# facebookresearch/dmc-net

Measured on AMD Instinct MI355X. Metric: clips/sec (3-seg 224x224) DMC-gen+ResNet-18 train step, higher is better.
Workload: dtype f32

## Files before the change

### dmc-net_amd/csrc/conv_x3q.hip

```cpp
#include "dmc_common.h"
#include "x3s_common.h"
#include <type_traits>
#include <utility>

using namespace dmc;
using namespace dmc::x3;

namespace {

constexpr int QBM = 256, QBN = 64;
constexpr int QWSLOT = 3 * QBN * 32;
constexpr int QWB = 3 * QWSLOT;
constexpr int QEP = 272, QETILE = 32 * QEP;

template <int NW_, int NPB_, int NT_>
struct QG {
    static constexpr int NW = NW_, NPB = NPB_, NT = NT_;
    static constexpr int NA = NW / 2;
    static constexpr int KP = (NT + NA - 1) / NA;
    static constexpr int PT = 3 * KP;
    static constexpr int KW = (18 + NA - 1) / NA;
    static constexpr int ZROW = 32 * NT;
    static constexpr int PSL = (ZROW + 1) * 32;
    static constexpr int PB = 3 * PSL;
// ... 453 lines not shown

template <int TN, class GEO>
int launch_q_eval(const X3qEvalArgs& a, hipStream_t s) {
    static LdsLimit lim;
    const hipError_t attr = lim.raise(reinterpret_cast<const void*>(&x3q_conv_kernel<ProgFwd, TN, GEO, true>), GEO::LDS);
    if (attr != hipSuccess) return fail(DMC_E_LAUNCH, "x3q_conv_bn_eval: cannot raise the dynamic LDS limit: %s", hipGetErrorString(attr));
    constexpr int BM = 32 * GEO::NW / (2 / TN);
    dim3 grid((a.M + BM - 1) / BM, a.R / QBN);
    x3q_conv_kernel<ProgFwd, TN, GEO, true><<<grid, GEO::NW * 64, GEO::LDS, s>>>(a);
    return check_launch("x3q_conv_bn_eval");
}

int q_patch_pixels_max128(long M, int W);
int q_variant(long M, int W, int R) {
    const int forced = option(OPT_CONV_CFG);
    const bool two_ok = q_patch_pixels_max128(M, W) <= QGTwo::ZROW;
    if (forced == 201) return 0;
    if (forced == 202) return 1;
    if (forced == 203 && two_ok) return 2;
    if (forced != 204 && two_ok && ((M + 127) / 128) * (R / QBN) >= 512) return 2;
    return q_choose_tn(M, R) == 2 ? 0 : 1;
}
int q_block_pixels(int variant) { return variant == 0 ? 256 : 128; }


struct X3qWgArgs {
    const void* xq;
    const void* dys;
    float* part;
    int N, OH, Cin, Cout;
    unsigned plane_bytes;
    int steps, per_group, tiles_ci;
};

template <int OW_, int R, int HP_>
struct QWgGeom {
    static constexpr int PW = OW_ + 1;
    static constexpr int D1 = 3, D0 = 2;
    static constexpr int XPL1 = ((D1 * R * PW + 3) / 8) * 8 + 4;
    static constexpr int XPL0 = ((D0 * R * PW + 3) / 8) * 8 + 4;
    static constexpr int NPX = R * OW_;
    static constexpr int NKB = (NPX + 15) / 16;
    static constexpr int DYT = ((NKB * 16 + 31) / 32) * 32;
    static constexpr int DYPL = ((DYT + 3) / 8) * 8 + 4;
    static constexpr int XI = (R * PW + 31) / 32;
    static constexpr int DI = DYT / 32;
    static constexpr int CLS_OFF[4] = {0, 4 * XPL0 * 32, 8 * XPL0 * 32, 8 * XPL0 * 32 + 4 * XPL1 * 32};
    static constexpr int SLB = 8 * XPL0 * 32 + 8 * XPL1 * 32;
    static constexpr int XBYTES = 3 * SLB, DYBYTES = 12 * DYPL * 32;
    static constexpr int LDS = XBYTES + 2 * DYBYTES;
    static_assert(HP_ % R == 0, "steps are whole groups of padded rows");
};

template <int OW_, int R, int HP_>
__global__ __launch_bounds__(768) void x3q_wgrad_kernel(X3qWgArgs a) {
    using G = QWgGeom<OW_, R, HP_>;
    constexpr int PW = G::PW, DYPL = G::DYPL, NKB = G::NKB;
    extern __shared__ __attribute__((aligned(1024))) char lds_qw[];
    const int tid = threadIdx.x, lane = tid & 63;
    const int wave = __builtin_amdgcn_readfirstlane(tid >> 6);
    const int l31 = lane & 31, khalf = lane >> 5, L = lane & 15, grp = (lane >> 4) & 1;
    const int quarter = wave & 3, trow = wave >> 2;
    const int wi = quarter & 1, wj = quarter >> 1;
    const int tci = blockIdx.x % a.tiles_ci, tco = blockIdx.x / a.tiles_ci;
    const unsigned lds0 = lds_addr_of(lds_qw);
    const int s_begin = blockIdx.y * a.per_group;
    const int s_end = s_begin + a.per_group < a.steps ? s_begin + a.per_group : a.steps;
    const u32x4 srd_x = make_srd(a.xq), srd_d = make_srd(a.dys);
    const int nch_in = a.Cin >> 4;
    const int tsl = wave >> 2, tch = wave & 3;
    const unsigned soff_d = (unsigned)(tsl * (a.Cout >> 4) + tco * 4 + tch) * a.plane_bytes;
    const unsigned dplane = lds0 + G::XBYTES + (unsigned)wave * DYPL * 32;
    const int lpx = lane >> 1;
    const unsigned lhalf = (unsigned)(lane & 1) << 4;

    const unsigned img_bytes = (unsigned)(a.OH * OW_) * 32u;
    unsigned xpre[G::XI], dpre[G::DI];
#pragma unroll
    for (int i = 0; i < G::XI; ++i) {
        const int px = 32 * i + lpx;
        const int r = px / PW, col = px - r * PW - 1;
        xpre[i] = (col >= 0 && col < OW_) ? (unsigned)(r * OW_ + col) * 32u + lhalf : NOPIX;
    }
#pragma unroll
    for (int i = 0; i < G::DI; ++i) {
        const int p = 32 * i + lpx;
        dpre[i] = p < G::NPX ? (unsigned)p * 32u + lhalf : NOPIX;
    }
    auto issue_x = [&](int q, const WgGroupPos& g) {
        unsigned tbase, img_off;
        wg_group_base(g, a.N, OW_, img_bytes, tbase, img_off);
        unsigned voff[G::XI];
#pragma unroll
        for (int i = 0; i < G::XI; ++i) voff[i] = wg_lane_off(tbase, xpre[i], img_bytes);
#pragma unroll
        for (int cls = 0; cls < 4; ++cls) {
            const int D = (cls >> 1) ? G::D1 : G::D0, xpl = (cls >> 1) ? G::XPL1 : G::XPL0;
            const int slot0 = (((q % D) + D) % D) * R;
            const unsigned soff_x = (unsigned)(tsl * 4 * nch_in + cls * nch_in + tci * 4 + tch) * a.plane_bytes + img_off;
            const unsigned xplane = lds0 + (unsigned)(tsl * G::SLB + G::CLS_OFF[cls] + tch * xpl * 32);
#pragma unroll
            for (int i = 0; i < G::XI; ++i)
                if (32 * i + lpx < R * PW) dma_buf16(srd_x, voff[i], soff_x, xplane + (unsigned)(slot0 * PW + 32 * i) * 32u);
        }
    };
    auto issue_dy = [&](const WgGroupPos& g, int buf) {
        unsigned tbase, img_off;
        wg_group_base(g, a.N, OW_, img_bytes, tbase, img_off);
#pragma unroll
        for (int i = 0; i < G::DI; ++i)
            dma_buf16(srd_d, wg_lane_off(tbase, dpre[i], img_bytes), soff_d + img_off, dplane + (unsigned)buf * G::DYBYTES + (unsigned)(32 * i) * 32u);
    };

    f32x16 acc[3];
#pragma unroll
    for (int t = 0; t < 3; ++t)
#pragma unroll
        for (int e = 0; e < 16; ++e) acc[t][e] = 0.f;

    WgGroupPos g1 = wg_group_at(s_begin, R, HP_);
    if (s_begin < s_end) {
        issue_x(s_begin - 1, wg_group_prev(g1, R, HP_));
        issue_x(s_begin, g1);
        issue_dy(g1, 0);
    }
    g1 = wg_group_next(g1, R, HP_);
    asm volatile("s_waitcnt vmcnt(0)" ::: "memory");
    __builtin_amdgcn_s_barrier();
    const int py = trow != 1, da = trow == 0 ? -1 : 0;
    const int DR = (py ? G::D1 : G::D0) * R, xpl = py ? G::XPL1 : G::XPL0;
    const int cls_a = py ? G::CLS_OFF[3] : G::CLS_OFF[1];
    const int cls_b = py ? G::CLS_OFF[2] : G::CLS_OFF[0];
    lds_cptr const LB = (lds_cptr)lds_qw;
    int rr[NKB][2], xcol[NKB][2], dyoff[NKB][2];
#pragma unroll
    for (int kb = 0; kb < NKB; ++kb)
#pragma unroll
        for (int u = 0; u < 2; ++u) {
            int P = 16 * kb + 8 * khalf + 4 * u + (L >> 2);
            dyoff[kb][u] = (2 * wi + grp) * DYPL * 32 + G::XBYTES + (L & 3) * 8 + P * 32;
            if (P >= G::NPX) P = G::NPX - 1;
            rr[kb][u] = P / OW_;
            xcol[kb][u] = (2 * wj + grp) * xpl * 32 + (L & 3) * 8 + (P - rr[kb][u] * OW_) * 32;
        }
#pragma unroll 1
    for (int s = s_begin; s < s_end; ++s) {
        const int buf = (s - s_begin) & 1;
        issue_x(s + 1, g1);
        if (s + 1 < s_end) issue_dy(g1, buf ^ 1);
        g1 = wg_group_next(g1, R, HP_);
        const int sb = (((R * s + da) % DR) + DR) % DR;
#pragma unroll
        for (int kb = 0; kb < NKB; ++kb) {
            int dyo[2], xa[2], xb[2];
#pragma unroll
            for (int u = 0; u < 2; ++u) {
                dyo[u] = dyoff[kb][u] + buf * G::DYBYTES;
                int slot = sb + rr[kb][u];
                slot = slot >= DR ? slot - DR : slot;
                const int xo = xcol[kb][u] + slot * PW * 32;
                xa[u] = xo + cls_a;
                xb[u] = xo + cls_b;
            }
            u32x4 A[3], B[3][3];
#pragma unroll
            for (int sl = 0; sl < 3; ++sl) {
                A[sl] = tr_read2(LB + dyo[0] + sl * 4 * DYPL * 32, LB + dyo[1] + sl * 4 * DYPL * 32);
                B[0][sl] = tr_read2(LB + xa[0] + sl * G::SLB, LB + xa[1] + sl * G::SLB);
                B[1][sl] = tr_read2(LB + xb[0] + sl * G::SLB + 32, LB + xb[1] + sl * G::SLB + 32);
                B[2][sl] = tr_read2(LB + xa[0] + sl * G::SLB + 32, LB + xa[1] + sl * G::SLB + 32);
            }
#pragma unroll
            for (int t = 0; t < 3; ++t) {
                acc[t] = mfma_bf16(A[0], B[t][2], acc[t]);
                acc[t] = mfma_bf16(A[2], B[t][0], acc[t]);
                acc[t] = mfma_bf16(A[1], B[t][1], acc[t]);
                acc[t] = mfma_bf16(A[0], B[t][1], acc[t]);
                acc[t] = mfma_bf16(A[1], B[t][0], acc[t]);
                acc[t] = mfma_bf16(A[0], B[t][0], acc[t]);
            }
        }
        asm volatile("s_waitcnt vmcnt(0) lgkmcnt(0)" ::: "memory");
        __builtin_amdgcn_s_barrier();
    }
    float* out = a.part + (size_t)blockIdx.y * a.Cout * 9 * a.Cin;
    const int ci = tci * 64 + 32 * wj + l31;
#pragma unroll
    for (int t = 0; t < 3; ++t)
#pragma unroll
        for (int e = 0; e < 16; ++e) {
            const int co = tco * 64 + 32 * wi + 8 * (e >> 2) + 4 * khalf + (e & 3);
            out[((size_t)co * 9 + 3 * trow + t) * a.Cin + ci] = acc[t][e];
        }
}

struct X3qWg1Args {
    const void* xq; const void* dys; float* part;
    int Cin, Cout; long Mq; unsigned plane_bytes; int steps, per_group, tiles_ci;
};
constexpr int W1PX = 64, W1PL = 68;
constexpr int W1TILE = 12 * W1PL * 32, W1LDS = 4 * W1TILE;

__global__ __launch_bounds__(256) void x3q_wgrad1_kernel(X3qWg1Args a) {
    extern __shared__ __attribute__((aligned(1024))) char lds_w1[];
    const int tid = threadIdx.x, lane = tid & 63;
    const int wave = __builtin_amdgcn_readfirstlane(tid >> 6);
    const int l31 = lane & 31, khalf = lane >> 5, L = lane & 15, grp = (lane >> 4) & 1;
    const int wi = wave & 1, wj = wave >> 1;
    const int tci = blockIdx.x % a.tiles_ci, tco = blockIdx.x / a.tiles_ci;
    const unsigned lds0 = lds_addr_of(lds_w1);
    const int s_begin = blockIdx.y * a.per_group;
    const int s_end = s_begin + a.per_group < a.steps ? s_begin + a.per_group : a.steps;
    const u32x4 srd_x = make_srd(a.xq), srd_d = make_srd(a.dys);
    const int nch_in = a.Cin >> 4, nch_out = a.Cout >> 4;
    const int lpx = lane >> 1;
    const unsigned lhalf = (unsigned)(lane & 1) << 4;
    auto issue = [&](int s, int buf) {
#pragma unroll
        for (int k = 0; k < 3; ++k) {
            const int pl = 3 * wave + k, sl = pl >> 2, ch = pl & 3;
#pragma unroll
            for (int i = 0; i < 2; ++i) {
                const long p = (long)s * W1PX + 32 * i + lpx;
                const unsigned voff = p < a.Mq ? (unsigned)p * 32u + lhalf : OOB;
                dma_buf16(srd_x, voff, (unsigned)(sl * 4 * nch_in + tci * 4 + ch) * a.plane_bytes,
                          lds0 + (unsigned)(buf * 2 * W1TILE + pl * W1PL * 32 + 32 * i * 32));
                dma_buf16(srd_d, voff, (unsigned)(sl * nch_out + tco * 4 + ch) * a.plane_bytes,
                          lds0 + (unsigned)(buf * 2 * W1TILE + W1TILE + pl * W1PL * 32 + 32 * i * 32));
            }
        }
    };
    f32x16 acc;
#pragma unroll
    for (int e = 0; e < 16; ++e) acc[e] = 0.f;
    if (s_begin < s_end) issue(s_begin, 0);
    asm volatile("s_waitcnt vmcnt(0)" ::: "memory");
// ... 11 lines not shown
            const int P0 = 16 * kb + 8 * khalf + (L >> 2), P1 = P0 + 4;
#pragma unroll
            for (int sl = 0; sl < 3; ++sl) {
                A[sl] = tr_read2(LB + db + sl * 4 * W1PL * 32 + P0 * 32, LB + db + sl * 4 * W1PL * 32 + P1 * 32);
                B[sl] = tr_read2(LB + xb + sl * 4 * W1PL * 32 + P0 * 32, LB + xb + sl * 4 * W1PL * 32 + P1 * 32);
            }
            acc = mfma_bf16(A[0], B[2], acc);
            acc = mfma_bf16(A[2], B[0], acc);
            acc = mfma_bf16(A[1], B[1], acc);
            acc = mfma_bf16(A[0], B[1], acc);
            acc = mfma_bf16(A[1], B[0], acc);
            acc = mfma_bf16(A[0], B[0], acc);
        }
        asm volatile("s_waitcnt vmcnt(0) lgkmcnt(0)" ::: "memory");
        __builtin_amdgcn_s_barrier();
    }
    float* out = a.part + (size_t)blockIdx.y * a.Cout * a.Cin;
    const int ci = tci * 64 + 32 * wj + l31;
#pragma unroll
    for (int e = 0; e < 16; ++e) {
        const int co = tco * 64 + 32 * wi + 8 * (e >> 2) + 4 * khalf + (e & 3);
        out[(size_t)co * a.Cin + ci] = acc[e];
    }
}

__global__ __launch_bounds__(256) void x3q_wgrad_reduce_kernel(const float* __restrict__ part, float* __restrict__ dw, int ngroup, long numel) {
    for (long i0 = (long)blockIdx.x * 64; i0 < numel; i0 += (long)gridDim.x * 64) wgrad_reduce_step(part, dw, ngroup, numel, i0);
}

struct QWgPlan { int R, HP, steps, tiles, groups, per_group, steps1, groups1, per_group1; };
bool q_wgrad_plan(int N, int OH, int OW, int Cin, int Cout, QWgPlan& p) {
    if (Cin % 64 != 0 || Cout % 64 != 0 || N <= 0) return false;
    if (OW == 28 && OH == 28) { p.R = 1; p.HP = 29; }
    else if (OW == 14 && OH == 14) { p.R = 2; p.HP = 16; }
    else if (OW == 7 && OH == 7) { p.R = 4; p.HP = 8; }
    else return false;
    p.steps = N * p.HP / p.R;
    p.tiles = (Cout / 64) * (Cin / 64);
    int groups = 256 / p.tiles;
    if (groups < 1) groups = 1;
    if (groups > p.steps) groups = p.steps;
    p.per_group = (p.steps + groups - 1) / groups;
    p.groups = (p.steps + p.per_group - 1) / p.per_group;
    const long Mq = (long)N * OH * OW;
    p.steps1 = (int)((Mq + W1PX - 1) / W1PX);
    int g1 = 512 / p.tiles;
    if (g1 < 1) g1 = 1;
    if (g1 > p.steps1) g1 = p.steps1;
    p.per_group1 = (p.steps1 + g1 - 1) / g1;
    p.groups1 = (p.steps1 + p.per_group1 - 1) / p.per_group1;
    return true;
}

template <int OW_, int R, int HP_>
int launch_q_wgrad(const QWgPlan& p, const X3qWgArgs& a, hipStream_t s) {
    using G = QWgGeom<OW_, R, HP_>;
    static_assert(G::LDS <= 160 * 1024, "weight-gradient tiles exceed the LDS");
    static LdsLimit lim;
    const hipError_t attr = lim.raise(reinterpret_cast<const void*>(&x3q_wgrad_kernel<OW_, R, HP_>), G::LDS);
    if (attr != hipSuccess) return fail(DMC_E_LAUNCH, "x3q_wgrad: cannot raise the dynamic LDS limit: %s", hipGetErrorString(attr));
    x3q_wgrad_kernel<OW_, R, HP_><<<dim3(p.tiles, p.groups), 768, G::LDS, s>>>(a);
    return check_launch("x3q_wgrad");
}

}

extern "C" {

size_t dmc_x3q_wpack_bytes(int Cin, int Cout) { return (size_t)Cin * (size_t)Cout * 10 * 6; }

int dmc_x3q_supported(int N, int OH, int OW, int Cin, int Cout) { return q_shape_ok(N, OH, OW, Cin, Cout) ? 1 : 0; }

int dmc_x3q_stat_blocks(int N, int OH, int OW, int Cout) {
    const long M = (long)N * OH * OW;
    const int bm = q_block_pixels(q_variant(M, OW, Cout));
    return (int)((M + bm - 1) / bm);
}

int dmc_x3q_split(const float* x, void* xq, int N, int H, int W, int C, dmc_stream_t stream) {
    if (!x || !xq || N <= 0 || H <= 0 || W <= 0 || (H & 1) || (W & 1) || C <= 0 || C % 16 != 0)
        return fail(DMC_E_INVALID, "dmc_x3q_split: bad argument");
    x3q_split_kernel<<<stream_blocks_q((long)N * H * W * (C / 8)), 256, 0, (hipStream_t)stream>>>(x, static_cast<unsigned short*>(xq), N, H, W, C);
    return check_launch("x3q_split");
}

int dmc_x3q_merge(const void* xq, float* x, int N, int H, int W, int C, dmc_stream_t stream) {
    if (!x || !xq || N <= 0 || H <= 0 || W <= 0 || (H & 1) || (W & 1) || C <= 0 || C % 16 != 0)
        return fail(DMC_E_INVALID, "dmc_x3q_merge: bad argument");
    x3q_merge_kernel<<<stream_blocks_q((long)N * H * W * C), 256, 0, (hipStream_t)stream>>>(static_cast<const unsigned short*>(xq), x, N, H, W, C);
    return check_launch("x3q_merge");
}

int dmc_x3q_pack_weights(const float* w3, const float* w1, void* wpack_f, void* wpack_t, int Cin, int Cout, dmc_stream_t stream) {
    if (!w3 || !w1 || (!wpack_f && !wpack_t) || Cin % 64 != 0 || Cout % 64 != 0 || Cin <= 0 || Cout <= 0)
        return fail(DMC_E_INVALID, "dmc_x3q_pack_weights: bad argument");
    const long total = (long)Cin * Cout * 10;
    const int blocks = stream_blocks_q(total) > 1024 ? 1024 : stream_blocks_q(total);
    x3q_pack_w_kernel<<<dim3(blocks, 2), 256, 0, (hipStream_t)stream>>>(w3, w1, static_cast<unsigned short*>(wpack_f),
                                                                           static_cast<unsigned short*>(wpack_t), Cout, Cin);
    return check_launch("x3q_pack_w");
}

int dmc_x3q_conv_fwd(const void* xq, const void* wpack_f, float* y3, float* y1, double* stat_partials3, double* stat_partials1,
                     int stat_blocks, int N, int OH, int OW, int Cin, int Cout, dmc_stream_t stream) {
    if (!xq || !wpack_f || !y3 || !y1) return fail(DMC_E_INVALID, "dmc_x3q_conv_fwd: null pointer");
    if (!q_shape_ok(N, OH, OW, Cin, Cout))
        return fail(DMC_E_INVALID, "dmc_x3q_conv_fwd: unsupported shape N=%d OH=%d OW=%d Cin=%d Cout=%d", N, OH, OW, Cin, Cout);
    const int var = q_variant((long)N * OH * OW, OW, Cout);
    const int rows = (int)(((long)N * OH * OW + q_block_pixels(var) - 1) / q_block_pixels(var));
    if ((stat_partials3 || stat_partials1) && stat_blocks != rows)
        return fail(DMC_E_INVALID, "dmc_x3q_conv_fwd: statistics partials have %d rows but this launch writes %d (dmc_x3q_stat_blocks "
                                   "was called under another conv_cfg option?)", stat_blocks, rows);
    X3qArgs a;
    a.t0 = xq; a.t1 = nullptr; a.wp = wpack_f; a.y0 = y3; a.y1 = y1; a.part0 = stat_partials3; a.part1 = stat_partials1;
    a.N = N; a.H = OH; a.W = OW; a.K = Cin; a.R = Cout; a.M = N * OH * OW;
// ... 89 lines not shown
```

### dmc-net_amd/csrc/conv_x3s.hip

```cpp
#include "dmc_common.h"
#include "x3s_common.h"
#include <type_traits>

using namespace dmc;
using namespace dmc::x3;

namespace {

__global__ __launch_bounds__(256) void x3s_split_kernel(const float* __restrict__ x, unsigned short* __restrict__ xs, long M, int C) {
    const int c8 = C >> 3;
    const long total = M * c8;
    const int nchunk = C >> 4;
    for (long o = (long)blockIdx.x * 256 + threadIdx.x; o < total; o += (long)gridDim.x * 256) {
        const long m = o / c8;
        const int g = (int)(o - m * c8);
        const float4 a = reinterpret_cast<const float4*>(x)[2 * o], b = reinterpret_cast<const float4*>(x)[2 * o + 1];
        const float v[8] = {a.x, a.y, a.z, a.w, b.x, b.y, b.z, b.w};
        x3s_store8(xs, v, (size_t)M, nchunk, (size_t)m, g);
    }
}

__global__ __launch_bounds__(256) void x3s_merge_kernel(const unsigned short* __restrict__ xs, float* __restrict__ x, long M, int C) {
    const long total = M * C;
    const size_t plane = (size_t)M * 16;
// ... 574 lines not shown
}

struct X3Bnb { const float *y, *stats, *gamma, *beta; const unsigned char* mask; int relu; double* part; };

int run_x3s(const void* xs, const void* wp, const float* addend, float* y, double* stat_part, int part_blocks, int N, int H, int W,
            int K, int R, hipStream_t s, const X3Bnb* bnb = nullptr) {
    if (!xs || !wp || !y) return fail(DMC_E_INVALID, "x3s_conv: null pointer");
    if (!x3s_shape_ok(N, H, W, K, R)) return fail(DMC_E_INVALID, "x3s_conv: unsupported shape N=%d H=%d W=%d K=%d R=%d", N, H, W, K, R);
    const int cfg = x3s_choose(N, H, W, R);
    X3Args a;
    a.xs = xs; a.wp = wp; a.y = y; a.addend = addend; a.stat_part = stat_part;
    a.N = N; a.H = H; a.W = W; a.K = K; a.R = R; a.M = N * H * W;
    a.plane_bytes = (unsigned)a.M * 32u;
    a.part_blocks = part_blocks;
    a.bms = cfg >= 0 ? x3s_tile_stride(cfg, W) : 0;
    if ((stat_part || bnb) && part_blocks <= 0) return fail(DMC_E_INVALID, "x3s_conv: stat_blocks must be the row count of the partials");
    if (bnb) {
        a.bnb_y = bnb->y; a.bnb_stats = bnb->stats; a.bnb_gamma = bnb->gamma; a.bnb_beta = bnb->beta; a.bnb_mask = bnb->mask;
        a.bnb_relu = bnb->relu; a.bnb_part = bnb->part;
    }
    a.ablate = option(OPT_CONV_ABLATE);
    if (DMC_ABL(a.ablate) & 32) a.stat_part = nullptr;
    switch (cfg) {
        case 0: return launch_x3s<8, 1, 608>(a, s);
        case 1: return launch_x3s<4, 1, 320>(a, s);
        case 2: return launch_x3s<2, 1, 192>(a, s);
        case 3: return launch_x3s<4, 2, 608>(a, s);
        case 4: return launch_x3s<4, 1, 225>(a, s);
        case 5: return launch_x3s<8, 2, 640, true>(a, s);
        default: return fail(DMC_E_INVALID, "x3s_conv: the patch of a %d x %d image does not fit the LDS", H, W);
    }
}

template <int WM, int TM, int PPMAX, bool ROWT = false>
int launch_x3s_eval(const X3EvalArgs& a, hipStream_t s) {
    constexpr int BM = 32 * TM * WM;
    constexpr size_t lds_bytes = 2 * 3 * PPMAX * 32 + 2 * 3 * 3 * 64 * 32;
    static_assert((size_t)BM * 272 <= lds_bytes && lds_bytes <= 160 * 1024, "the epilogue tiles live in the operand LDS");
    dim3 grid((a.M + a.bms - 1) / a.bms, a.R / 64);
    static LdsLimit lim_attr;
    const hipError_t attr = lim_attr.raise(reinterpret_cast<const void*>(&x3s_conv_kernel<WM, 1, TM, 2, PPMAX, (WM >= 4), 1, true, ROWT>), (int)lds_bytes);
    if (attr != hipSuccess) return fail(DMC_E_LAUNCH, "x3s_conv_bn_eval: cannot raise the dynamic LDS limit: %s", hipGetErrorString(attr));
    x3s_conv_kernel<WM, 1, TM, 2, PPMAX, (WM >= 4), 1, true, ROWT><<<grid, WM * 64, lds_bytes, s>>>(a);
    return check_launch("x3s_conv_bn_eval");
}

struct X3WgArgs {
    const void* xs;
    const void* dys;
    float* part;
    int N, H, Cin, Cout;
    unsigned plane_bytes;
    int steps, per_group, tiles_ci;
};

template <int W_, int R>
struct WgGeom {
    static constexpr int PW = W_ + 2;
    static constexpr int NGRP = R >= W_ + 2 ? 2 : 4, LA = NGRP / 2;
    static constexpr int NRING = NGRP * R;
    static constexpr int XPX = NRING * PW;
    static constexpr int XPL = ((XPX + 3) / 8) * 8 + 4;
    static constexpr int NPX = R * W_;
    static constexpr int NKB = (NPX + 15) / 16;
    static constexpr int DYP = NKB * 16;
    static constexpr int DYT = ((DYP + 31) / 32) * 32;
    static constexpr int DYPL = ((DYT + 3) / 8) * 8 + 4;
    static constexpr int XI = (R * PW + 31) / 32;
    static constexpr int DI = DYT / 32;
    static constexpr int XBYTES = 12 * XPL * 32, DYBYTES = 12 * DYPL * 32;
    static constexpr int LDS = XBYTES + 2 * DYBYTES;
};

template <int W_, int R>
__global__ __launch_bounds__(768) void x3s_wgrad_kernel(X3WgArgs a) {
    using G = WgGeom<W_, R>;
    constexpr int PW = G::PW, NRING = G::NRING, XPL = G::XPL, DYPL = G::DYPL, NKB = G::NKB;
    extern __shared__ __attribute__((aligned(1024))) char lds_wg[];
    const int tid = threadIdx.x, lane = tid & 63;
    const int wave = __builtin_amdgcn_readfirstlane(tid >> 6);
    const int l31 = lane & 31, khalf = lane >> 5, L = lane & 15, grp = (lane >> 4) & 1;
    const int quarter = wave & 3, trow = wave >> 2;
    const int wi = quarter & 1, wj = quarter >> 1;
    const int tci = blockIdx.x % a.tiles_ci, tco = blockIdx.x / a.tiles_ci;
    const unsigned lds0 = lds_addr_of(lds_wg);
    const int HP = a.H + 2;
    const int s_begin = blockIdx.y * a.per_group;
    const int s_end = s_begin + a.per_group < a.steps ? s_begin + a.per_group : a.steps;
    const u32x4 srd_x = make_srd(a.xs), srd_d = make_srd(a.dys);
    const unsigned soff_x = (unsigned)((wave >> 2) * (a.Cin >> 4) + tci * 4 + (wave & 3)) * a.plane_bytes;
    const unsigned soff_d = (unsigned)((wave >> 2) * (a.Cout >> 4) + tco * 4 + (wave & 3)) * a.plane_bytes;
    const unsigned xplane = lds0 + (unsigned)wave * XPL * 32, dplane = lds0 + G::XBYTES + (unsigned)wave * DYPL * 32;
    const int lpx = lane >> 1;
    const unsigned lhalf = (unsigned)(lane & 1) << 4;

    const unsigned img_bytes = (unsigned)(a.H * W_) * 32u;
    unsigned xpre[G::XI], dpre[G::DI];
#pragma unroll
    for (int i = 0; i < G::XI; ++i) {
        const int px = 32 * i + lpx;
        const int r = px / PW, col = px - r * PW - 1;
        xpre[i] = (col >= 0 && col < W_) ? (unsigned)(r * W_ + col) * 32u + lhalf : NOPIX;
    }
#pragma unroll
    for (int i = 0; i < G::DI; ++i) {
        const int p = 32 * i + lpx;
        dpre[i] = p < G::NPX ? (unsigned)p * 32u + lhalf : NOPIX;
    }
    auto issue_x = [&](int q, const WgGroupPos& g) {
        const int slot0 = (((q % G::NGRP) + G::NGRP) % G::NGRP) * R;
        unsigned tbase, img_off;
        wg_group_base(g, a.N, W_, img_bytes, tbase, img_off);
#pragma unroll
        for (int i = 0; i < G::XI; ++i)
            if (32 * i + lpx < R * PW)
                dma_buf16(srd_x, wg_lane_off(tbase, xpre[i], img_bytes), soff_x + img_off, xplane + (unsigned)(slot0 * PW + 32 * i) * 32u);
    };
    auto issue_dy = [&](const WgGroupPos& g, int buf) {
        unsigned tbase, img_off;
        wg_group_base(g, a.N, W_, img_bytes, tbase, img_off);
#pragma unroll
        for (int i = 0; i < G::DI; ++i)
            dma_buf16(srd_d, wg_lane_off(tbase, dpre[i], img_bytes), soff_d + img_off, dplane + (unsigned)buf * G::DYBYTES + (unsigned)(32 * i) * 32u);
    };

    f32x16 acc[3];
#pragma unroll
    for (int t = 0; t < 3; ++t)
#pragma unroll
        for (int e = 0; e < 16; ++e) acc[t][e] = 0.f;

    WgGroupPos g1 = wg_group_at(s_begin, R, HP);
    if (s_begin < s_end) {
        WgGroupPos g = wg_group_prev(g1, R, HP);
#pragma unroll
        for (int q = -1; q < G::LA; ++q, g = wg_group_next(g, R, HP)) issue_x(s_begin + q, g);
        issue_dy(g1, 0);
    }
    g1 = wg_group_next(g1, R, HP);
    asm volatile("s_waitcnt vmcnt(0)" ::: "memory");
    __builtin_amdgcn_s_barrier();
    lds_cptr const LB = (lds_cptr)lds_wg;
    int rr[NKB][2], xcol[NKB][2], dyoff[NKB][2];
#pragma unroll
    for (int kb = 0; kb < NKB; ++kb)
#pragma unroll
        for (int u = 0; u < 2; ++u) {
            int P = 16 * kb + 8 * khalf + 4 * u + (L >> 2);
            dyoff[kb][u] = (2 * wi + grp) * DYPL * 32 + G::XBYTES + (L & 3) * 8 + P * 32;
            if (P >= G::NPX) P = G::NPX - 1;
            rr[kb][u] = P / W_;
            xcol[kb][u] = (2 * wj + grp) * XPL * 32 + (L & 3) * 8 + (P - rr[kb][u] * W_) * 32;
        }
#pragma unroll 1
    for (int s = s_begin; s < s_end; ++s) {
        const int buf = (s - s_begin) & 1;
        issue_x(s + G::LA, G::LA == 1 ? g1 : wg_group_next(g1, R, HP));
        if (s + 1 < s_end) issue_dy(g1, buf ^ 1);
        g1 = wg_group_next(g1, R, HP);
        const int sb = (((R * s + trow - 1) % NRING) + NRING) % NRING;
#pragma unroll
        for (int kb = 0; kb < NKB; ++kb) {
            int dyo[2], xo[2];
#pragma unroll
            for (int u = 0; u < 2; ++u) {
                dyo[u] = dyoff[kb][u] + buf * G::DYBYTES;
                int slot = sb + rr[kb][u];
                slot = slot >= NRING ? slot - NRING : slot;
                xo[u] = xcol[kb][u] + slot * PW * 32;
            }
            u32x4 A[3], B[3][3];
#pragma unroll
            for (int sl = 0; sl < 3; ++sl) {
                A[sl] = tr_read2(LB + dyo[0] + sl * 4 * DYPL * 32, LB + dyo[1] + sl * 4 * DYPL * 32);
#pragma unroll
                for (int t = 0; t < 3; ++t)
                    B[t][sl] = tr_read2(LB + xo[0] + (sl * 4 * XPL + t) * 32, LB + xo[1] + (sl * 4 * XPL + t) * 32);
            }
#pragma unroll
            for (int t = 0; t < 3; ++t) {
                acc[t] = mfma_bf16(A[0], B[t][2], acc[t]);
                acc[t] = mfma_bf16(A[2], B[t][0], acc[t]);
                acc[t] = mfma_bf16(A[1], B[t][1], acc[t]);
                acc[t] = mfma_bf16(A[0], B[t][1], acc[t]);
                acc[t] = mfma_bf16(A[1], B[t][0], acc[t]);
                acc[t] = mfma_bf16(A[0], B[t][0], acc[t]);
            }
        }
        asm volatile("s_waitcnt vmcnt(0) lgkmcnt(0)" ::: "memory");
        __builtin_amdgcn_s_barrier();
    }
    float* out = a.part + (size_t)blockIdx.y * a.Cout * 9 * a.Cin;
    const int ci = tci * 64 + 32 * wj + l31;
#pragma unroll
    for (int t = 0; t < 3; ++t)
#pragma unroll
        for (int e = 0; e < 16; ++e) {
            const int co = tco * 64 + 32 * wi + 8 * (e >> 2) + 4 * khalf + (e & 3);
            out[((size_t)co * 9 + 3 * trow + t) * a.Cin + ci] = acc[t][e];
        }
}

__global__ __launch_bounds__(256) void x3s_wgrad_reduce_kernel(const float* __restrict__ part, float* __restrict__ dw, int ngroup, long numel) {
    for (long i0 = (long)blockIdx.x * 64; i0 < numel; i0 += (long)gridDim.x * 64) wgrad_reduce_step(part, dw, ngroup, numel, i0);
}

struct X3WgPlan { int R, steps, tiles, groups, per_group; };
bool x3s_wgrad_plan(int N, int H, int W, int Cin, int Cout, X3WgPlan& p) {
    p.R = W == 56 ? 1 : W == 28 ? 2 : W == 14 ? 4 : W == 7 ? 9 : 0;
    if (!p.R || (H + 2) % p.R != 0 || (W == 7 && H != 7) || Cin % 64 != 0 || Cout % 64 != 0) return false;
    p.steps = N * (H + 2) / p.R;
    p.tiles = (Cout / 64) * (Cin / 64);
    int groups = 256 / p.tiles;
    if (groups < 1) groups = 1;
    if (groups > p.steps) groups = p.steps;
    p.per_group = (p.steps + groups - 1) / groups;
    p.groups = (p.steps + p.per_group - 1) / p.per_group;
    return true;
}

template <int W_, int R>
int launch_x3s_wgrad(const X3WgPlan& p, X3WgArgs a, float* dw, hipStream_t s) {
    using G = WgGeom<W_, R>;
    static_assert(G::LDS <= 160 * 1024, "weight-gradient tiles exceed the LDS");
    static LdsLimit lim_attr;
    const hipError_t attr = lim_attr.raise(reinterpret_cast<const void*>(&x3s_wgrad_kernel<W_, R>), G::LDS);
    if (attr != hipSuccess) return fail(DMC_E_LAUNCH, "x3s_wgrad: cannot raise the dynamic LDS limit: %s", hipGetErrorString(attr));
    x3s_wgrad_kernel<W_, R><<<dim3(p.tiles, p.groups), 768, G::LDS, s>>>(a);
    int rc = check_launch("x3s_wgrad");
    if (rc || p.groups == 1) return rc;
    const long numel = (long)a.Cout * 9 * a.Cin;
    const long blocks = (numel + 63) / 64;
    x3s_wgrad_reduce_kernel<<<(int)(blocks > 4096 ? 4096 : blocks), 256, 0, s>>>(a.part, dw, p.groups, numel);
    return check_launch("x3s_wgrad_reduce");
}

__global__ __launch_bounds__(256) void x3s_bnb_final_kernel(const double* __restrict__ part, int nblk, int C,
                                                            float* __restrict__ dgamma, float* __restrict__ dbeta) {
    __shared__ double red[2][4];
    const int c = blockIdx.x, lane = threadIdx.x & 63, wave = threadIdx.x >> 6;
    double s = 0.0, ss = 0.0;
    for (int b = threadIdx.x; b < nblk; b += 256) {
        const double2 v = *reinterpret_cast<const double2*>(part + ((size_t)b * C + c) * 2);
        s += v.x;
        ss += v.y;
    }
#pragma unroll
    for (int o = 32; o > 0; o >>= 1) { s += __shfl_down(s, o, 64); ss += __shfl_down(ss, o, 64); }
    if (lane == 0) { red[0][wave] = s; red[1][wave] = ss; }
    __syncthreads();
    if (threadIdx.x != 0) return;
    dbeta[c] = (float)(red[0][0] + red[0][1] + red[0][2] + red[0][3]);
    dgamma[c] = (float)(red[1][0] + red[1][1] + red[1][2] + red[1][3]);
}

int stream_blocks(long total) {
    long b = (total + 255) / 256;
    return (int)(b < 1 ? 1 : (b > 8192 ? 8192 : b));
}

}

extern "C" {

size_t dmc_x3s_slices_bytes(long M, int C) { return (size_t)M * (size_t)C * 6; }

int dmc_x3s_split(const float* x, void* xs, long M, int C, dmc_stream_t stream) {
    if (!x || !xs || M <= 0 || C <= 0 || C % 16 != 0) return fail(DMC_E_INVALID, "dmc_x3s_split: bad argument");
    x3s_split_kernel<<<stream_blocks(M * (C / 8)), 256, 0, (hipStream_t)stream>>>(x, static_cast<unsigned short*>(xs), M, C);
    return check_launch("x3s_split");
}

int dmc_x3s_merge(const void* xs, float* x, long M, int C, dmc_stream_t stream) {
    if (!x || !xs || M <= 0 || C <= 0 || C % 16 != 0) return fail(DMC_E_INVALID, "dmc_x3s_merge: bad argument");
    x3s_merge_kernel<<<stream_blocks(M * C), 256, 0, (hipStream_t)stream>>>(static_cast<const unsigned short*>(xs), x, M, C);
    return check_launch("x3s_merge");
}

size_t dmc_x3s_wpack_bytes(int Cin, int Cout) { return (size_t)Cin * (size_t)Cout * 9 * 6; }

int dmc_x3s_pack_weights(const float* w, void* wpack_f, void* wpack_t, int Cin, int Cout, dmc_stream_t stream) {
    if (!w || (!wpack_f && !wpack_t) || Cin % 64 != 0 || Cout % 64 != 0 || Cin <= 0 || Cout <= 0)
// ... 141 lines not shown
```

### dmc-net_amd/csrc/x3s_common.h

```cpp
#pragma once
#include "dmc_common.h"

namespace dmc {
namespace x3 {

constexpr unsigned NOPIX = 0x40000000u;

struct WgGroupPos { int n, y; };
__device__ __forceinline__ WgGroupPos wg_group_at(int q, int R, int HP) {
    const int g = R * q, n = g / HP;
    WgGroupPos p;
    p.n = __builtin_amdgcn_readfirstlane(n);
    p.y = __builtin_amdgcn_readfirstlane(g - n * HP);
    return p;
}
__device__ __forceinline__ WgGroupPos wg_group_next(WgGroupPos p, int R, int HP) {
    p.y += R;
    if (p.y >= HP) { p.y -= HP; ++p.n; }
    return p;
}
__device__ __forceinline__ WgGroupPos wg_group_prev(WgGroupPos p, int R, int HP) {
    p.y -= R;
    if (p.y < 0) { p.y += HP; --p.n; }
    return p;
}
__device__ __forceinline__ void wg_group_base(const WgGroupPos& p, int N, int W, unsigned img_bytes, unsigned& tbase, unsigned& img_off) {
    const bool in = p.n >= 0 && p.n < N;
    tbase = in ? (unsigned)((p.y - 1) * W) * 32u : NOPIX;
    img_off = in ? (unsigned)p.n * img_bytes : 0u;
}
__device__ __forceinline__ unsigned wg_lane_off(unsigned tbase, unsigned pre, unsigned img_bytes) {
    const unsigned t = tbase + pre;
    return t < img_bytes ? t : OOB;
}

}
}
```

Before: 3574.

## Software-pipeline LDS fragment reads under MFMAs in 3x3 weight-gradient kernels

Replaces the per-step read-all-then-multiply loop in the x3s and x3q weight-gradient kernels with a software-pipelined step. The next fragment's LDS transposed reads are interleaved between the MFMAs of the current one, pinned in place by sched_barriers. Ring offsets are now advanced incrementally instead of recomputed with modulo, and the global prefetch plus barrier are moved to the step tail. In x3s, k-blocks whose rows fall entirely in the zero padding at the image top or bottom skip their MFMAs. The old loop is kept behind a config option, and a DMC_MEASURE-only timing-stamp variant is added. This holds more fragments live in registers and depends on careful ordering around the dy buffer switch.

```diff
diff --git a/dmc-net_amd/csrc/conv_x3q.hip b/dmc-net_amd/csrc/conv_x3q.hip
--- a/dmc-net_amd/csrc/conv_x3q.hip
+++ b/dmc-net_amd/csrc/conv_x3q.hip
@@ -529,7 +529,8 @@
     static_assert(HP_ % R == 0, "steps are whole groups of padded rows");
 };
 
-template <int OW_, int R, int HP_>
+constexpr int X3Q_WG_CFG_PARENT_LOOP = 109;
+template <int OW_, int R, int HP_, int LOOP>
 __global__ __launch_bounds__(768) void x3q_wgrad_kernel(X3qWgArgs a) {
     using G = QWgGeom<OW_, R, HP_>;
     constexpr int PW = G::PW, DYPL = G::DYPL, NKB = G::NKB;
@@ -620,45 +621,111 @@
             rr[kb][u] = P / OW_;
             xcol[kb][u] = (2 * wj + grp) * xpl * 32 + (L & 3) * 8 + (P - rr[kb][u] * OW_) * 32;
         }
+    auto mfma6 = [&](f32x16& c, const u32x4 (&A)[3], const u32x4 (&B)[3]) {
+        c = mfma_bf16(A[0], B[2], c);
+        c = mfma_bf16(A[2], B[0], c);
+        c = mfma_bf16(A[1], B[1], c);
+        c = mfma_bf16(A[0], B[1], c);
+        c = mfma_bf16(A[1], B[0], c);
+        c = mfma_bf16(A[0], B[0], c);
+    };
+    if constexpr (LOOP == 0) {
+        const int STEPB = R * PW * 32, RINGB = DR * PW * 32, dcls = cls_b - cls_a;
+        int ring[NKB][2];
+        {
+            const int sb = (((R * s_begin + da) % DR) + DR) % DR;
+#pragma unroll
+            for (int kb = 0; kb < NKB; ++kb)
+#pragma unroll
+                for (int u = 0; u < 2; ++u) {
+                    int slot = sb + (R == 1 ? 0 : rr[kb][u]);
+                    slot = slot >= DR ? slot - DR : slot;
+                    ring[kb][u] = slot * PW * 32 + cls_a;
+                }
+        }
+        int dyb = 0;
+        auto read_a = [&](int kb, int sl) {
+            return tr_read2(LB + dyoff[kb][0] + dyb + sl * 4 * DYPL * 32, LB + dyoff[kb][1] + dyb + sl * 4 * DYPL * 32);
+        };
+        auto read_b = [&](int kb, int t, int sl) {
+            const int o = (t == 1 ? dcls : 0) + sl * G::SLB + (t == 0 ? 0 : 32);
+            return tr_read2(LB + xcol[kb][0] + ring[kb][0] + o, LB + xcol[kb][1] + ring[kb][1] + o);
+        };
+        auto issue_ahead = [&](int s) {
+            if (s + 1 < s_end) {
+                issue_x(s + 1, g1);
+                issue_dy(g1, ((s - s_begin) & 1) ^ 1);
+            }
+            g1 = wg_group_next(g1, R, HP_);
+        };
+        auto boundary = [&]() {
+            asm volatile("s_waitcnt vmcnt(0)" ::: "memory");
+            __builtin_amdgcn_s_waitcnt(0xC07F);
+            __builtin_amdgcn_s_barrier();
+        };
+        u32x4 A0[2], A1, A2, B0[2], B1, B2;
+        if (s_begin < s_end) {
+            issue_ahead(s_begin);
+            A0[0] = read_a(0, 0); A2 = read_a(0, 2); A1 = read_a(0, 1);
+            B2 = read_b(0, 0, 2); B0[0] = read_b(0, 0, 0); B1 = read_b(0, 0, 1);
+        }
+        auto step = [&](int s, auto more_c) {
+            constexpr bool MORE = decltype(more_c)::value;
+            wg_step_pipelined<NKB, MORE>(
+                acc, A0, A1, A2, B0, B1, B2, read_a, read_b, boundary,
+                [&](int kb, int t) {
+                    if (!MORE) return;
+                    if (kb == NKB - 2 && t == 2) dyb = G::DYBYTES - dyb;
+                    if (kb == NKB - 1 && t == 1) {
+#pragma unroll
+                        for (int k2 = 0; k2 < NKB; ++k2)
+#pragma unroll
+                            for (int u = 0; u < 2; ++u) {
+                                const int nx = ring[k2][u] + STEPB;
+                                ring[k2][u] = nx >= RINGB + cls_a ? nx - RINGB : nx;
+                            }
+                    }
+                    if (kb == NKB - 1 && t == 2) issue_ahead(s + 1);
+                },
+                [](int) { return false; });
+        };
 #pragma unroll 1
-    for (int s = s_begin; s < s_end; ++s) {
-        const int buf = (s - s_begin) & 1;
-        issue_x(s + 1, g1);
-        if (s + 1 < s_end) issue_dy(g1, buf ^ 1);
-        g1 = wg_group_next(g1, R, HP_);
-        const int sb = (((R * s + da) % DR) + DR) % DR;
-#pragma unroll
-        for (int kb = 0; kb < NKB; ++kb) {
-            int dyo[2], xa[2], xb[2];
-#pragma unroll
-            for (int u = 0; u < 2; ++u) {
-                dyo[u] = dyoff[kb][u] + buf * G::DYBYTES;
-                int slot = sb + rr[kb][u];
-                slot = slot >= DR ? slot - DR : slot;
-                const int xo = xcol[kb][u] + slot * PW * 32;
-                xa[u] = xo + cls_a;
-                xb[u] = xo + cls_b;
-            }
-            u32x4 A[3], B[3][3];
-#pragma unroll
-            for (int sl = 0; sl < 3; ++sl) {
-                A[sl] = tr_read2(LB + dyo[0] + sl * 4 * DYPL * 32, LB + dyo[1] + sl * 4 * DYPL * 32);
-                B[0][sl] = tr_read2(LB + xa[0] + sl * G::SLB, LB + xa[1] + sl * G::SLB);
-                B[1][sl] = tr_read2(LB + xb[0] + sl * G::SLB + 32, LB + xb[1] + sl * G::SLB + 32);
-                B[2][sl] = tr_read2(LB + xa[0] + sl * G::SLB + 32, LB + xa[1] + sl * G::SLB + 32);
-            }
-#pragma unroll
-            for (int t = 0; t < 3; ++t) {
-                acc[t] = mfma_bf16(A[0], B[t][2], acc[t]);
-                acc[t] = mfma_bf16(A[2], B[t][0], acc[t]);
-                acc[t] = mfma_bf16(A[1], B[t][1], acc[t]);
-                acc[t] = mfma_bf16(A[0], B[t][1], acc[t]);
-                acc[t] = mfma_bf16(A[1], B[t][0], acc[t]);
-                acc[t] = mfma_bf16(A[0], B[t][0], acc[t]);
-            }
-        }
-        asm volatile("s_waitcnt vmcnt(0) lgkmcnt(0)" ::: "memory");
-        __builtin_amdgcn_s_barrier();
+        for (int s = s_begin; s + 1 < s_end; ++s) step(s, std::true_type{});
+        if (s_begin < s_end) step(s_end - 1, std::false_type{});
+    } else {
+#pragma unroll 1
+        for (int s = s_begin; s < s_end; ++s) {
+            const int buf = (s - s_begin) & 1;
+            issue_x(s + 1, g1);
+            if (s + 1 < s_end) issue_dy(g1, buf ^ 1);
+            g1 = wg_group_next(g1, R, HP_);
+            const int sb = (((R * s + da) % DR) + DR) % DR;
+#pragma unroll
+            for (int kb = 0; kb < NKB; ++kb) {
+                int dyo[2], xa[2], xb[2];
+#pragma unroll
+                for (int u = 0; u < 2; ++u) {
+                    dyo[u] = dyoff[kb][u] + buf * G::DYBYTES;
+                    int slot = sb + rr[kb][u];
+                    slot = slot >= DR ? slot - DR : slot;
+                    const int xo = xcol[kb][u] + slot * PW * 32;
+                    xa[u] = xo + cls_a;
+                    xb[u] = xo + cls_b;
+                }
+                u32x4 A[3], B[3][3];
+#pragma unroll
+                for (int sl = 0; sl < 3; ++sl) {
+                    A[sl] = tr_read2(LB + dyo[0] + sl * 4 * DYPL * 32, LB + dyo[1] + sl * 4 * DYPL * 32);
+                    B[0][sl] = tr_read2(LB + xa[0] + sl * G::SLB, LB + xa[1] + sl * G::SLB);
+                    B[1][sl] = tr_read2(LB + xb[0] + sl * G::SLB + 32, LB + xb[1] + sl * G::SLB + 32);
+                    B[2][sl] = tr_read2(LB + xa[0] + sl * G::SLB + 32, LB + xa[1] + sl * G::SLB + 32);
+                }
+#pragma unroll
+                for (int t = 0; t < 3; ++t) mfma6(acc[t], A, B[t]);
+            }
+            asm volatile("s_waitcnt vmcnt(0) lgkmcnt(0)" ::: "memory");
+            __builtin_amdgcn_s_barrier();
+        }
     }
     float* out = a.part + (size_t)blockIdx.y * a.Cout * 9 * a.Cin;
     const int ci = tci * 64 + 32 * wj + l31;
@@ -776,15 +843,19 @@
     return true;
 }
 
-template <int OW_, int R, int HP_>
-int launch_q_wgrad(const QWgPlan& p, const X3qWgArgs& a, hipStream_t s) {
+template <int OW_, int R, int HP_, int LOOP>
+int launch_q_wgrad_loop(const QWgPlan& p, const X3qWgArgs& a, hipStream_t s) {
     using G = QWgGeom<OW_, R, HP_>;
     static_assert(G::LDS <= 160 * 1024, "weight-gradient tiles exceed the LDS");
     static LdsLimit lim;
-    const hipError_t attr = lim.raise(reinterpret_cast<const void*>(&x3q_wgrad_kernel<OW_, R, HP_>), G::LDS);
+    const hipError_t attr = lim.raise(reinterpret_cast<const void*>(&x3q_wgrad_kernel<OW_, R, HP_, LOOP>), G::LDS);
     if (attr != hipSuccess) return fail(DMC_E_LAUNCH, "x3q_wgrad: cannot raise the dynamic LDS limit: %s", hipGetErrorString(attr));
-    x3q_wgrad_kernel<OW_, R, HP_><<<dim3(p.tiles, p.groups), 768, G::LDS, s>>>(a);
+    x3q_wgrad_kernel<OW_, R, HP_, LOOP><<<dim3(p.tiles, p.groups), 768, G::LDS, s>>>(a);
     return check_launch("x3q_wgrad");
+}
+template <int OW_, int R, int HP_>
+int launch_q_wgrad(const QWgPlan& p, const X3qWgArgs& a, hipStream_t s) {
+    return option(OPT_CONV_CFG) == X3Q_WG_CFG_PARENT_LOOP ? launch_q_wgrad_loop<OW_, R, HP_, 1>(p, a, s) : launch_q_wgrad_loop<OW_, R, HP_, 0>(p, a, s);
 }
 
 }
diff --git a/dmc-net_amd/csrc/conv_x3s.hip b/dmc-net_amd/csrc/conv_x3s.hip
--- a/dmc-net_amd/csrc/conv_x3s.hip
+++ b/dmc-net_amd/csrc/conv_x3s.hip
@@ -650,7 +650,21 @@
     int N, H, Cin, Cout;
     unsigned plane_bytes;
     int steps, per_group, tiles_ci;
+#ifdef DMC_MEASURE
+    unsigned long long* stamps;
+#endif
 };
+constexpr int X3S_WG_CFG_PARENT_LOOP = 109;
+
+#ifdef DMC_MEASURE
+__device__ __forceinline__ unsigned long long wg_stamp() {
+    unsigned long long t;
+    __builtin_amdgcn_sched_barrier(0);
+    asm volatile("s_memtime %0\n\ts_waitcnt lgkmcnt(0)" : "=s"(t) :: "memory");
+    __builtin_amdgcn_sched_barrier(0);
+    return t;
+}
+#endif
 
 template <int W_, int R>
 struct WgGeom {
@@ -670,7 +684,7 @@
     static constexpr int LDS = XBYTES + 2 * DYBYTES;
 };
 
-template <int W_, int R>
+template <int W_, int R, int LOOP>
 __global__ __launch_bounds__(768) void x3s_wgrad_kernel(X3WgArgs a) {
     using G = WgGeom<W_, R>;
     constexpr int PW = G::PW, NRING = G::NRING, XPL = G::XPL, DYPL = G::DYPL, NKB = G::NKB;
@@ -750,43 +764,150 @@
             rr[kb][u] = P / W_;
             xcol[kb][u] = (2 * wj + grp) * XPL * 32 + (L & 3) * 8 + (P - rr[kb][u] * W_) * 32;
         }
+    auto mfma6 = [&](f32x16& c, const u32x4 (&A)[3], const u32x4 (&B)[3]) {
+        c = mfma_bf16(A[0], B[2], c);
+        c = mfma_bf16(A[2], B[0], c);
+        c = mfma_bf16(A[1], B[1], c);
+        c = mfma_bf16(A[0], B[1], c);
+        c = mfma_bf16(A[1], B[0], c);
+        c = mfma_bf16(A[0], B[0], c);
+    };
+    if constexpr (LOOP == 0) {
+        static_assert(NKB >= 2, "the dy buffer is switched behind the reads of the last k-block's A fragments");
+        constexpr int STEPB = R * PW * 32, RINGB = NRING * PW * 32;
+        int ring[NKB][2];
+        {
+            const int sb = (((R * s_begin + trow - 1) % NRING) + NRING) % NRING;
+#pragma unroll
+            for (int kb = 0; kb < NKB; ++kb)
+#pragma unroll
+                for (int u = 0; u < 2; ++u) {
+                    int slot = sb + (R == 1 ? 0 : rr[kb][u]);
+                    slot = slot >= NRING ? slot - NRING : slot;
+                    ring[kb][u] = slot * PW * 32;
+                }
+        }
+        int dyb = 0;
+        auto read_a = [&](int kb, int sl) {
+            return tr_read2(LB + dyoff[kb][0] + dyb + sl * 4 * DYPL * 32, LB + dyoff[kb][1] + dyb + sl * 4 * DYPL * 32);
+        };
+        auto read_b = [&](int kb, int t, int sl) {
+            return tr_read2(LB + xcol[kb][0] + ring[kb][0] + (sl * 4 * XPL + t) * 32, LB + xcol[kb][1] + ring[kb][1] + (sl * 4 * XPL + t) * 32);
+        };
+        auto issue_ahead = [&](int s) {
+            if (s + 1 < s_end) {
+                issue_x(s + G::LA, G::LA == 1 ? g1 : wg_group_next(g1, R, HP));
+                issue_dy(g1, ((s - s_begin) & 1) ^ 1);
+            }
+            g1 = wg_group_next(g1, R, HP);
+        };
+        auto boundary = [&]() {
+            asm volatile("s_waitcnt vmcnt(0)" ::: "memory");
+            __builtin_amdgcn_s_waitcnt(0xC07F);
+            __builtin_amdgcn_s_barrier();
+        };
+        u32x4 A0[2], A1, A2, B0[2], B1, B2;
+        if (s_begin < s_end) {
+            issue_ahead(s_begin);
+            A0[0] = read_a(0, 0); A2 = read_a(0, 2); A1 = read_a(0, 1);
+            B2 = read_b(0, 0, 2); B0[0] = read_b(0, 0, 0); B1 = read_b(0, 0, 1);
+        }
+        int ycur = __builtin_amdgcn_readfirstlane((R * s_begin) % HP);
+        auto step = [&](int s, auto more_c) {
+            constexpr bool MORE = decltype(more_c)::value;
+            const bool first_grp = ycur == 0, last_grp = ycur == HP - R;
+            ycur = ycur + R >= HP ? ycur + R - HP : ycur + R;
+            wg_step_pipelined<NKB, MORE>(
+                acc, A0, A1, A2, B0, B1, B2, read_a, read_b, boundary,
+                [&](int kb, int t) {
+                    if (!MORE) return;
+                    if (kb == NKB - 2 && t == 2) dyb = G::DYBYTES - dyb;
+                    if (kb == NKB - 1 && t == 1) {
+#pragma unroll
+                        for (int k2 = 0; k2 < NKB; ++k2)
+#pragma unroll
+                            for (int u = 0; u < 2; ++u) {
+                                const int nx = ring[k2][u] + STEPB;
+                                ring[k2][u] = nx >= RINGB ? nx - RINGB : nx;
+                            }
+                    }
+                    if (kb == NKB - 1 && t == 2) issue_ahead(s + 1);
+                },
+                [&](int kb) {
+                    const int lo = (16 * kb) / W_, hi = (16 * kb + 15 < G::NPX ? 16 * kb + 15 : G::NPX - 1) / W_;
+                    return (lo == 0 && hi == 0 && first_grp) || (lo == R - 1 && hi == R - 1 && last_grp);
+                });
+        };
 #pragma unroll 1
-    for (int s = s_begin; s < s_end; ++s) {
-        const int buf = (s - s_begin) & 1;
-        issue_x(s + G::LA, G::LA == 1 ? g1 : wg_group_next(g1, R, HP));
-        if (s + 1 < s_end) issue_dy(g1, buf ^ 1);
-        g1 = wg_group_next(g1, R, HP);
-        const int sb = (((R * s + trow - 1) % NRING) + NRING) % NRING;
-#pragma unroll
-        for (int kb = 0; kb < NKB; ++kb) {
-            int dyo[2], xo[2];
-#pragma unroll
-            for (int u = 0; u < 2; ++u) {
-                dyo[u] = dyoff[kb][u] + buf * G::DYBYTES;
-                int slot = sb + rr[kb][u];
-                slot = slot >= NRING ? slot - NRING : slot;
-                xo[u] = xcol[kb][u] + slot * PW * 32;
+        for (int s = s_begin; s + 1 < s_end; ++s) step(s, std::true_type{});
+        if (s_begin < s_end) step(s_end - 1, std::false_type{});
+    } else {
+#ifdef DMC_MEASURE
+        [[maybe_unused]] unsigned long long st_issue = 0, st_read = 0, st_wait = 0, st_mfma = 0, st_drain = 0, st_cal = 0, st_t0 = 0, st_t = 0;
+        if constexpr (LOOP == 2) {
+            st_t0 = wg_stamp();
+            st_t = wg_stamp();
+            st_cal = st_t - st_t0;
+            st_t0 = st_t;
+        }
+#endif
+#pragma unroll 1
+        for (int s = s_begin; s < s_end; ++s) {
+            const int buf = (s - s_begin) & 1;
+            issue_x(s + G::LA, G::LA == 1 ? g1 : wg_group_next(g1, R, HP));
+            if (s + 1 < s_end) issue_dy(g1, buf ^ 1);
+            g1 = wg_group_next(g1, R, HP);
+            const int sb = (((R * s + trow - 1) % NRING) + NRING) % NRING;
+#ifdef DMC_MEASURE
+            if constexpr (LOOP == 2) { const unsigned long long t = wg_stamp(); st_issue += t - st_t; st_t = t; }
+#endif
+#pragma unroll
+            for (int kb = 0; kb < NKB; ++kb) {
+                int dyo[2], xo[2];
+#pragma unroll
+                for (int u = 0; u < 2; ++u) {
+                    dyo[u] = dyoff[kb][u] + buf * G::DYBYTES;
+                    int slot = sb + rr[kb][u];
+                    slot = slot >= NRING ? slot - NRING : slot;
+                    xo[u] = xcol[kb][u] + slot * PW * 32;
+                }
+                u32x4 A[3], B[3][3];
+#pragma unroll
+                for (int sl = 0; sl < 3; ++sl) {
+                    A[sl] = tr_read2(LB + dyo[0] + sl * 4 * DYPL * 32, LB + dyo[1] + sl * 4 * DYPL * 32);
+#pragma unroll
+                    for (int t = 0; t < 3; ++t)
+                        B[t][sl] = tr_read2(LB + xo[0] + (sl * 4 * XPL + t) * 32, LB + xo[1] + (sl * 4 * XPL + t) * 32);
+                }
+#ifdef DMC_MEASURE
+                if constexpr (LOOP == 2) {
+                    unsigned long long t = wg_stamp();
+                    st_read += t - st_t; st_t = t;
+                    t = wg_stamp();
+                    st_wait += t - st_t; st_t = t;
+                }
+#endif
+#pragma unroll
+                for (int t = 0; t < 3; ++t) mfma6(acc[t], A, B[t]);
+#ifdef DMC_MEASURE
+                if constexpr (LOOP == 2) { const unsigned long long t = wg_stamp(); st_mfma += t - st_t; st_t = t; }
+#endif
             }
-            u32x4 A[3], B[3][3];
-#pragma unroll
-            for (int sl = 0; sl < 3; ++sl) {
-                A[sl] = tr_read2(LB + dyo[0] + sl * 4 * DYPL * 32, LB + dyo[1] + sl * 4 * DYPL * 32);
-#pragma unroll
-                for (int t = 0; t < 3; ++t)
-                    B[t][sl] = tr_read2(LB + xo[0] + (sl * 4 * XPL + t) * 32, LB + xo[1] + (sl * 4 * XPL + t) * 32);
+            asm volatile("s_waitcnt vmcnt(0) lgkmcnt(0)" ::: "memory");
+            __builtin_amdgcn_s_barrier();
+#ifdef DMC_MEASURE
+            if constexpr (LOOP == 2) { const unsigned long long t = wg_stamp(); st_drain += t - st_t; st_t = t; }
+#endif
+        }
+#ifdef DMC_MEASURE
+        if constexpr (LOOP == 2) {
+            if (lane == 0 && a.stamps != nullptr) {
+                unsigned long long* o = a.stamps + ((size_t)(blockIdx.y * gridDim.x + blockIdx.x) * 12 + wave) * 8;
+                o[0] = st_issue; o[1] = st_read; o[2] = st_wait; o[3] = st_mfma; o[4] = st_drain; o[5] = st_t - st_t0;
+                o[6] = st_cal; o[7] = (unsigned long long)(s_end - s_begin);
             }
-#pragma unroll
-            for (int t = 0; t < 3; ++t) {
-                acc[t] = mfma_bf16(A[0], B[t][2], acc[t]);
-                acc[t] = mfma_bf16(A[2], B[t][0], acc[t]);
-                acc[t] = mfma_bf16(A[1], B[t][1], acc[t]);
-                acc[t] = mfma_bf16(A[0], B[t][1], acc[t]);
-                acc[t] = mfma_bf16(A[1], B[t][0], acc[t]);
-                acc[t] = mfma_bf16(A[0], B[t][0], acc[t]);
-            }
-        }
-        asm volatile("s_waitcnt vmcnt(0) lgkmcnt(0)" ::: "memory");
-        __builtin_amdgcn_s_barrier();
+        }
+#endif
     }
     float* out = a.part + (size_t)blockIdx.y * a.Cout * 9 * a.Cin;
     const int ci = tci * 64 + 32 * wj + l31;
@@ -817,15 +938,27 @@
     return true;
 }
 
-template <int W_, int R>
-int launch_x3s_wgrad(const X3WgPlan& p, X3WgArgs a, float* dw, hipStream_t s) {
+template <int W_, int R, int LOOP>
+int launch_x3s_wgrad_loop(const X3WgPlan& p, const X3WgArgs& a, hipStream_t s) {
     using G = WgGeom<W_, R>;
     static_assert(G::LDS <= 160 * 1024, "weight-gradient tiles exceed the LDS");
     static LdsLimit lim_attr;
-    const hipError_t attr = lim_attr.raise(reinterpret_cast<const void*>(&x3s_wgrad_kernel<W_, R>), G::LDS);
+    const hipError_t attr = lim_attr.raise(reinterpret_cast<const void*>(&x3s_wgrad_kernel<W_, R, LOOP>), G::LDS);
     if (attr != hipSuccess) return fail(DMC_E_LAUNCH, "x3s_wgrad: cannot raise the dynamic LDS limit: %s", hipGetErrorString(attr));
-    x3s_wgrad_kernel<W_, R><<<dim3(p.tiles, p.groups), 768, G::LDS, s>>>(a);
-    int rc = check_launch("x3s_wgrad");
+    x3s_wgrad_kernel<W_, R, LOOP><<<dim3(p.tiles, p.groups), 768, G::LDS, s>>>(a);
+    return check_launch("x3s_wgrad");
+}
+
+template <int W_, int R>
+int launch_x3s_wgrad(const X3WgPlan& p, X3WgArgs a, float* dw, hipStream_t s) {
+    int rc;
+#ifdef DMC_MEASURE
+    a.stamps = (option(OPT_CONV_ABLATE) & 2048) && p.groups > 1
+                   ? reinterpret_cast<unsigned long long*>(a.part + (size_t)p.groups * a.Cout * 9 * a.Cin) : nullptr;
+    if (a.stamps) rc = launch_x3s_wgrad_loop<W_, R, 2>(p, a, s);
+    else
+#endif
+    rc = option(OPT_CONV_CFG) == X3S_WG_CFG_PARENT_LOOP ? launch_x3s_wgrad_loop<W_, R, 1>(p, a, s) : launch_x3s_wgrad_loop<W_, R, 0>(p, a, s);
     if (rc || p.groups == 1) return rc;
     const long numel = (long)a.Cout * 9 * a.Cin;
     const long blocks = (numel + 63) / 64;
diff --git a/dmc-net_amd/csrc/x3s_common.h b/dmc-net_amd/csrc/x3s_common.h
--- a/dmc-net_amd/csrc/x3s_common.h
+++ b/dmc-net_amd/csrc/x3s_common.h
@@ -34,5 +34,46 @@
     return t < img_bytes ? t : OOB;
 }
 
+template <int NKB, bool MORE, class RA, class RB, class BD, class TL, class SK>
+__device__ __forceinline__ void wg_step_pipelined(f32x16 (&acc)[3], u32x4 (&A0)[2], u32x4& A1, u32x4& A2, u32x4 (&B0)[2], u32x4& B1,
+                                                  u32x4& B2, RA read_a, RB read_b, BD boundary, TL tail, SK skip) {
+    static_assert(NKB % 2 == 0, "A0 / B0 alternate with period 2 and a step must end on the registers it began with");
+#pragma unroll
+    for (int kb = 0; kb < NKB; ++kb) {
+        const bool zero = skip(kb);
+#pragma unroll
+        for (int t = 0; t < 3; ++t) {
+            const int i = 3 * kb + t;
+            const bool last = kb == NKB - 1 && t == 2;
+            const bool next = !last || MORE;
+            const int nkb = last ? 0 : (t == 2 ? kb + 1 : kb), nt = t == 2 ? 0 : t + 1;
+            const bool na = next && t == 2;
+            f32x16& c = acc[t];
+            if (last && MORE) boundary();
+            if (next) B0[(i + 1) & 1] = read_b(nkb, nt, 0);
+            if (na) A0[nkb & 1] = read_a(nkb, 0);
+            __builtin_amdgcn_sched_barrier(0);
+            if (!zero) c = mfma_bf16(A0[kb & 1], B2, c);
+            if (next) B2 = read_b(nkb, nt, 2);
+            __builtin_amdgcn_sched_barrier(0);
+            if (!zero) c = mfma_bf16(A2, B0[i & 1], c);
+            if (na) A2 = read_a(nkb, 2);
+            __builtin_amdgcn_sched_barrier(0);
+            if (!zero) {
+                c = mfma_bf16(A1, B1, c);
+                c = mfma_bf16(A0[kb & 1], B1, c);
+            }
+            if (next) B1 = read_b(nkb, nt, 1);
+            __builtin_amdgcn_sched_barrier(0);
+            if (!zero) c = mfma_bf16(A1, B0[i & 1], c);
+            if (na) A1 = read_a(nkb, 1);
+            __builtin_amdgcn_sched_barrier(0);
+            if (!zero) c = mfma_bf16(A0[kb & 1], B0[i & 1], c);
+            tail(kb, t);
+            __builtin_amdgcn_sched_barrier(0);
+        }
+    }
+}
+
 }
 }
```

Result: no change. 3572 (-0.1%).
